# jesselasse/MARL-DMFB

Measured on AMD Instinct MI355X. Metric: env-steps/sec (whole node), 10x10 DMFB 4-droplet fov9, higher is better.
Workload: dtype int8 env state/obs + f64 rewards; fp32 Q-net; 1 GPU; DMFB 10x10, drop_num=4, fov=9, 4096 parallel envs per GPU (BASELINE configs[1]); parallelism=dp1: chips sharded per rank, one flat RCCL all-reduce per learn

## Files before the change

### marl_dmfb_amd/_lib.py

```python
import ctypes as C
import os

_HERE = os.path.dirname(os.path.abspath(__file__))
LIB_DIR = os.path.join(_HERE, 'lib')
_CACHE = {}
_FILE = {'rollout_route': 'rollout_ops'}


class HipLibraryMissing(RuntimeError):
    pass


def load(name):
    if name in _CACHE:
        return _CACHE[name]
    stem = _FILE.get(name, name)
    path = os.path.join(LIB_DIR, 'lib%s%s.so' % (stem, os.environ.get('MARL_DMFB_VARIANT_' + stem.upper(), '')))
    if not os.path.exists(path):
        raise HipLibraryMissing(
            '%s not found: build the HIP extension first (python -c "import __graft_entry__ as g; g.build()" '
            'or make -C marl_dmfb_amd/csrc). There is no CPU fallback.' % path)
    import torch
    lib = C.CDLL(path)
    _CACHE[name] = lib
# ... 169 lines not shown
        'meda_plan_route': [i32, i32, i32, i32, vp, vp, vp, vp, vp, vp, vp, vp, vp, vp],
        'meda_plan_max_dim': ([], i32),
        'meda_plan_lds_bytes': ([i32, i32, i32], i32),
        'meda_plan_last_hip_error': ([], i32),
    },
    'vdn_ops': {
        'vdn_td_forward': [vp, vp, vp, vp, vp, vp, vp, i32, i32, i32, i32, i32, f32, vp, vp, vp, vp],
        'vdn_td_backward': [vp, vp, vp, vp, i32, i32, i32, i32, i32, vp, vp],
        'vdn_td_forward_packed': [vp, vp, vp, i32, vp, vp, vp, vp, vp, i32, i32, f32, vp, vp, vp, vp],
        'vdn_td_backward_packed': [vp, vp, vp, i32, vp, vp, i32, i32, vp, vp],
        'vdn_gather_units': [vp, i32, vp, i32, i32, i32, vp, vp],
        'vdn_clip_adam_step': [i32, C.POINTER(vp), C.POINTER(vp), C.POINTER(vp), C.POINTER(vp), C.POINTER(i64), f32, f64, f64, f64,
                               f64, f64, f64, vp, vp, vp, vp],
        'vdn_last_hip_error': ([], i32),
    },
    'qmix_ops': {
        'qmix_mix_td_forward': [vp, vp, vp, vp, vp, vp, vp, i32, i32, i32, i32, i32, vp, i32, i32, vp, i32, i32, i32, i32,
                                C.POINTER(QmixMixer), C.POINTER(QmixMixer), f32, vp, vp, vp, vp],
        'qmix_mix_td_backward': [vp, vp, vp, vp, i32, i32, i32, i32, i32, vp, i32, i32, i32, i32, C.POINTER(QmixMixer), vp, vp, vp,
                                 vp, vp, vp],
        'qmix_last_hip_error': ([], i32),
    },
}

DMFB_VEC_SYMBOLS = list(SIGNATURES['dmfb_vec'])
MEDA_VEC_SYMBOLS = list(SIGNATURES['meda_vec'])

ENV_ERRORS = {
    'dmfb_vec': {
        -1: (ValueError, 'bad argument'),
# ... 103 lines not shown
    return _library('rollout_route')


def route_plan():
    return _library('route_plan')


def meda_plan():
    return _library('meda_plan')


def vdn_ops():
    return _library('vdn_ops')


def qmix_ops():
    return _library('qmix_ops')
```

### marl_dmfb_amd/csrc/crnn_ops.hip

```cpp
#include <hip/hip_runtime.h>

#include <cstdint>
#include <cstdio>
#include <cstdlib>

#include "../../include/crnn_ops.h"

#define HIP_ABI_TAG "crnn_ops"
#define HIP_ABI_ERR CRNN_ERR_HIP
#include "hip_abi.h"
#include "crnn_mfma.h"
#include "crnn_mfma19.h"
#include "crnn_bwd19.h"

namespace {

constexpr int kBlock = 512;
constexpr int kA1Stride = 52;
constexpr int kDz1Unit = 108;

constexpr int kLdsBudget = 158 * 1024;

template <int OD> struct GeoB {
    static constexpr int DZ2 = 28;
// ... 354 lines not shown
            for (; b + kRedY < n_part; b += 2 * kRedY) { a0 += part[(size_t)b * G::PART + off[k]]; a1 += part[(size_t)(b + kRedY) * G::PART + off[k]]; }
            if (b < n_part) a0 += part[(size_t)b * G::PART + off[k]];
            acc += a0 + a1;
        }
    }
    s_sum[ty][tx] = acc;
    __syncthreads();
    if (ty == 0 && i < n2 + nb + n1 + nb) {
        float t = 0.0f;
#pragma unroll
        for (int k = 0; k < kRedY; ++k) t += s_sum[k][tx];
        grads[i] = t;
    }
}

constexpr int kMlpBlock = 256, kMlpOut = 10, kMlpMaxIn = 18, kMlpMaxParts = 256;
__global__ __launch_bounds__(kMlpBlock) void k_mlp_bwd(const int8_t *__restrict__ obs, long obs_stride, int dir_off,
                                                       const int8_t *__restrict__ onehot, int n_actions, long rows,
                                                       const float *__restrict__ x, long x_stride, const float *__restrict__ g, long g_stride,
                                                       int col0, float *__restrict__ part) {
    __shared__ float s_red[kMlpBlock / 64][kMlpOut * (kMlpMaxIn + 1)];
    float acc[kMlpOut][kMlpMaxIn + 1];
#pragma unroll
    for (int o = 0; o < kMlpOut; ++o)
#pragma unroll
        for (int k = 0; k <= kMlpMaxIn; ++k) acc[o][k] = 0.0f;
    for (long r = (long)blockIdx.x * kMlpBlock + threadIdx.x; r < rows; r += (long)gridDim.x * kMlpBlock) {
        float v[kMlpMaxIn];
        v[0] = (float)obs[r * obs_stride + dir_off];
        v[1] = (float)obs[r * obs_stride + dir_off + 1];
#pragma unroll
        for (int k = 0; k < kMlpMaxIn - 2; ++k) v[2 + k] = k < n_actions ? (float)onehot[r * n_actions + k] : 0.0f;
#pragma unroll
        for (int o = 0; o < kMlpOut; ++o) {
            const float gz = x[r * x_stride + col0 + o] > 0.0f ? g[r * g_stride + col0 + o] : 0.0f;
#pragma unroll
            for (int k = 0; k < kMlpMaxIn; ++k) acc[o][k] = fmaf(gz, v[k], acc[o][k]);
            acc[o][kMlpMaxIn] += gz;
        }
    }
    const int lane = threadIdx.x & 63, wave = threadIdx.x >> 6;
#pragma unroll
    for (int o = 0; o < kMlpOut; ++o)
#pragma unroll
        for (int k = 0; k <= kMlpMaxIn; ++k) {
            float t = acc[o][k];
            for (int d = 32; d > 0; d >>= 1) t += __shfl_xor(t, d);
            if (lane == 0) s_red[wave][o * (kMlpMaxIn + 1) + k] = t;
        }
    __syncthreads();
    for (int i = threadIdx.x; i < kMlpOut * (kMlpMaxIn + 1); i += kMlpBlock) {
        float t = 0.0f;
#pragma unroll
        for (int w = 0; w < kMlpBlock / 64; ++w) t += s_red[w][i];
        part[(size_t)blockIdx.x * kMlpOut * (kMlpMaxIn + 1) + i] = t;
    }
}
__global__ __launch_bounds__(256) void k_mlp_bwd_reduce(const float *__restrict__ part, int n_part, int nin, float *__restrict__ dw, float *__restrict__ db) {
    const int i = threadIdx.x;
    if (i >= kMlpOut * nin + kMlpOut) return;
    const int o = i < kMlpOut * nin ? i / nin : i - kMlpOut * nin, k = i < kMlpOut * nin ? i - o * nin : kMlpMaxIn;
    float t = 0.0f;
    for (int b = 0; b < n_part; ++b) t += part[(size_t)b * kMlpOut * (kMlpMaxIn + 1) + o * (kMlpMaxIn + 1) + k];
    if (i < kMlpOut * nin) dw[i] = t;
    else db[o] = t;
}

struct LiveRows { const int32_t *chips; const int32_t *n; int rows_per_chip; };

template <int OD, int RBV>
int launch_rb(const int8_t *obs, long obs_stride, long rows, const float *w1, const float *b1, const float *w2, const float *b2,
              float *out, long out_stride, int out_cols, const int8_t *onehot, int n_actions, const float *mlp_w, const float *mlp_b, hipStream_t s,
              LiveRows live = LiveRows{nullptr, nullptr, 1}) {
    using GM = crnn_mfma::GeoM<OD, RBV>;
    const size_t lds = GM::LDS_FLOATS * sizeof(float);
    static LdsLimit lds_limit;
    if (const int rc = lds_limit.raise((const void *)crnn_mfma::k_conv9_mfma<OD, RBV>, lds)) return rc;
    const long n_blocks = (rows + GM::RB - 1) / GM::RB;
    const long resident = 256L * (long)((size_t)160 * 1024 / lds);
    const int grid = (int)(n_blocks < resident ? n_blocks : resident);
// ... 128 lines not shown
    if (od == 32) return launch_bwd<32>(d_obs, obs_stride, rows, d_out, out_stride, d_grad_out, grad_stride, d_w2, d_part, n_part, d_grads, d_w1, d_b1, (hipStream_t)stream);
    return CRNN_ERR_UNSUPPORTED;
}

int crnn_mlp_backward_parts(void) { return kMlpMaxParts * kMlpOut * (kMlpMaxIn + 1); }

int crnn_mlp_backward(const int8_t *d_obs, int64_t obs_stride, int dir_offset, const int8_t *d_onehot, int n_actions, int64_t rows,
                      const float *d_out, int64_t out_stride, const float *d_grad_out, int64_t grad_stride, int col0, float *d_part,
                      float *d_grad_w, float *d_grad_b, void *stream) {
    if (!d_obs || !d_onehot || !d_out || !d_grad_out || !d_part || !d_grad_w || !d_grad_b || rows <= 0 || n_actions < 0 ||
        n_actions > kMlpMaxIn - 2 || dir_offset < 0 || obs_stride < dir_offset + 2 || col0 < 0 || out_stride < col0 + kMlpOut ||
        grad_stride < col0 + kMlpOut)
        return CRNN_ERR_BAD_ARG;
    const long want = (rows + kMlpBlock - 1) / kMlpBlock;
    const int grid = (int)(want < kMlpMaxParts ? want : kMlpMaxParts);
    HIP_TRY(launch_status([&] {
        hipLaunchKernelGGL(k_mlp_bwd, dim3(grid), dim3(kMlpBlock), 0, (hipStream_t)stream, d_obs, (long)obs_stride, dir_offset, d_onehot, n_actions,
                           (long)rows, d_out, (long)out_stride, d_grad_out, (long)grad_stride, col0, d_part);
        hipLaunchKernelGGL(k_mlp_bwd_reduce, dim3(1), dim3(256), 0, (hipStream_t)stream, d_part, grid, 2 + n_actions, d_grad_w, d_grad_b);
    }));
    return CRNN_OK;
}

int crnn_conv19_backward_parts(int od) { return od == 24 ? crnn_bwd19::GeoB19<24>::PART : od == 32 ? crnn_bwd19::GeoB19<32>::PART : CRNN_ERR_UNSUPPORTED; }

int crnn_conv19_backward(const int8_t *d_obs, int64_t obs_stride, int64_t rows, const float *d_out, int64_t out_stride,
                         const float *d_grad_out, int64_t grad_stride, const float *d_w1, const float *d_b1, const float *d_w3,
                         const float *d_b3, int od, float *d_part, int n_part, float *d_grads, void *stream) {
    if (!d_obs || !d_out || !d_grad_out || !d_w1 || !d_b1 || !d_w3 || !d_b3 || !d_part || !d_grads || rows <= 0 || n_part < 1 ||
        n_part > 256 || obs_stride < 3 * 19 * 19 || out_stride < od * 25 || grad_stride < od * 25)
        return CRNN_ERR_BAD_ARG;
    if (od == 24) return launch_bwd19<24>(d_obs, obs_stride, rows, d_out, out_stride, d_grad_out, grad_stride, d_w1, d_b1, d_w3, d_b3, d_part, n_part, d_grads, (hipStream_t)stream);
    if (od == 32) return launch_bwd19<32>(d_obs, obs_stride, rows, d_out, out_stride, d_grad_out, grad_stride, d_w1, d_b1, d_w3, d_b3, d_part, n_part, d_grads, (hipStream_t)stream);
    return CRNN_ERR_UNSUPPORTED;
}
// ... 5 lines not shown
```

### marl_dmfb_amd/csrc/hip_abi.h

```cpp
#pragma once

#include <hip/hip_runtime.h>

#include <cstdio>
#include <cstdlib>

#if !defined(HIP_ABI_TAG) || !defined(HIP_ABI_ERR)
#error "define HIP_ABI_TAG and HIP_ABI_ERR before including hip_abi.h"
#endif

namespace {

thread_local int g_last_hip = 0;

inline int hip_fail(hipError_t e, const char *what, int line) {
    g_last_hip = (int)e;
    if (getenv("DMFB_VEC_DEBUG"))
        fprintf(stderr, HIP_ABI_TAG ": %s failed at line %d: %s (%d)\n", what, line, hipGetErrorString(e), (int)e);
    return HIP_ABI_ERR;
}

#define HIP_TRY(expr)                                                 \
    do {                                                              \
        hipError_t _e = (expr);                                       \
// ... 30 lines not shown
};

struct LdsLimit {
    bool done[64] = {};
    int raise(const void *kernel, size_t bytes) {
        int dev = 0;
        (void)hipGetDevice(&dev);
        const bool known = dev >= 0 && dev < 64;
        if (known && done[dev]) return 0;
        HIP_TRY(hipFuncSetAttribute(kernel, hipFuncAttributeMaxDynamicSharedMemorySize, (int)bytes));
        if (known) done[dev] = true;
        return 0;
    }
};

}
```

### marl_dmfb_amd/csrc/vdn_ops.hip

```cpp
#include <hip/hip_runtime.h>

#include <cstdint>

#include "../../include/vdn_ops.h"

#define HIP_ABI_TAG "vdn_ops"
#define HIP_ABI_ERR VDN_ERR_HIP
#include "hip_abi.h"

namespace {

__global__ __launch_bounds__(256) void k_td_forward(const float *__restrict__ qe, const float *__restrict__ qt, const int8_t *__restrict__ u,
                                                    const float *__restrict__ r, const int8_t *__restrict__ avail,
                                                    const uint8_t *__restrict__ term, const uint8_t *__restrict__ padded, int B, int T,
                                                    int Tl, int n, int A, float gamma, float *__restrict__ mtd, float *__restrict__ maskf,
                                                    int32_t *__restrict__ bad) {
    const int idx = blockIdx.x * blockDim.x + threadIdx.x;
    if (idx >= B * T) return;
    const int b = idx / T, t = idx - b * T;
    const size_t ep = (size_t)b * Tl + t;
    const size_t q0 = ((size_t)t * B + b) * n * A;
    float qe_tot = 0.0f, qt_tot = 0.0f;
    bool ok = true;
    for (int i = 0; i < n; ++i) {
        int a_taken = (int)u[ep * n + i];
        if ((unsigned)a_taken >= (unsigned)A) { ok = false; a_taken = 0; }
        qe_tot = qe_tot + qe[q0 + (size_t)i * A + a_taken];
        float m = -3.4e38f;
        for (int a = 0; a < A; ++a) {
            const float v = avail[(ep * n + i) * A + a] == 0 ? -9999999.0f : qt[q0 + (size_t)i * A + a];
            m = v > m ? v : m;
        }
        qt_tot = qt_tot + m;
    }
    const float not_term = 1.0f - (term[ep] ? 1.0f : 0.0f);
    const float target = r[ep] + (gamma * qt_tot) * not_term;
    const float mk = 1.0f - (padded[ep] ? 1.0f : 0.0f);
    mtd[idx] = ok ? mk * (target - qe_tot) : __builtin_nanf("");
    maskf[idx] = mk;
    if (!ok && bad) atomicAdd(bad, 1);
}

__global__ __launch_bounds__(256) void k_td_backward(const float *__restrict__ mtd, const float *__restrict__ maskf, const int8_t *__restrict__ u,
                                                     const float *__restrict__ g, int B, int T, int Tl, int n, int A,
                                                     float *__restrict__ gq) {
    const long row = (long)blockIdx.x * blockDim.x + threadIdx.x;
    if (row >= (long)T * B * n) return;
    const int i = (int)(row % n);
    const long tb = row / n;
    const int b = (int)(tb % B), t = (int)(tb / B);
    const int idx = b * T + t;
    const float d = -((2.0f * mtd[idx]) * maskf[idx]) * g[0];
    const int a_taken = (int)u[((size_t)b * Tl + t) * n + i];
    const bool bad_a = (unsigned)a_taken >= (unsigned)A;
    for (int a = 0; a < A; ++a) gq[row * A + a] = (bad_a || a == a_taken) ? d : 0.0f;
}

__global__ __launch_bounds__(256) void k_td_forward_packed(const float *__restrict__ qe, const float *__restrict__ qt, const int32_t *__restrict__ units,
                                                           int U, const int8_t *__restrict__ u, const float *__restrict__ r,
                                                           const int8_t *__restrict__ avail, const uint8_t *__restrict__ term,
                                                           const uint8_t *__restrict__ padded, int n, int A, float gamma,
                                                           float *__restrict__ mtd, float *__restrict__ maskf, int32_t *__restrict__ bad) {
    const int j = blockIdx.x * blockDim.x + threadIdx.x;
    if (j >= U) return;
    const size_t ep = (size_t)units[j];
    const size_t q0 = (size_t)j * n * A;
    float qe_tot = 0.0f, qt_tot = 0.0f;
    bool ok = true;
    for (int i = 0; i < n; ++i) {
        int a_taken = (int)u[ep * n + i];
        if ((unsigned)a_taken >= (unsigned)A) { ok = false; a_taken = 0; }
        qe_tot = qe_tot + qe[q0 + (size_t)i * A + a_taken];
        float m = -3.4e38f;
        for (int a = 0; a < A; ++a) {
            const float v = avail[(ep * n + i) * A + a] == 0 ? -9999999.0f : qt[q0 + (size_t)i * A + a];
            m = v > m ? v : m;
        }
        qt_tot = qt_tot + m;
    }
    const float not_term = 1.0f - (term[ep] ? 1.0f : 0.0f);
    const float target = r[ep] + (gamma * qt_tot) * not_term;
    const float mk = 1.0f - (padded[ep] ? 1.0f : 0.0f);
    mtd[j] = ok ? mk * (target - qe_tot) : __builtin_nanf("");
    maskf[j] = mk;
    if (!ok && bad) atomicAdd(bad, 1);
}

__global__ __launch_bounds__(256) void k_td_backward_packed(const float *__restrict__ mtd, const float *__restrict__ maskf, const int32_t *__restrict__ units,
                                                            const int8_t *__restrict__ u, const float *__restrict__ g, long rows, int n, int A,
                                                            float *__restrict__ gq) {
    const long row = (long)blockIdx.x * blockDim.x + threadIdx.x;
    if (row >= rows) return;
    const int i = (int)(row % n);
    const long j = row / n;
    const float d = -((2.0f * mtd[j]) * maskf[j]) * g[0];
    const int a_taken = (int)u[(size_t)units[j] * n + i];
    const bool bad_a = (unsigned)a_taken >= (unsigned)A;
    for (int a = 0; a < A; ++a) gq[row * A + a] = (bad_a || a == a_taken) ? d : 0.0f;
}

template <typename V>
__global__ __launch_bounds__(256) void k_gather_units(const V *__restrict__ src, int unit_v, const int32_t *__restrict__ units, int U, int shift,
                                                      int zero_below, V *__restrict__ dst) {
    const long idx = (long)blockIdx.x * blockDim.x + threadIdx.x;
    if (idx >= (long)U * unit_v) return;
    const int j = (int)(idx / unit_v), k = (int)(idx - (long)j * unit_v);
    dst[idx] = j < zero_below ? (V)0 : src[((size_t)units[j] + shift) * unit_v + k];
}

}

namespace {

struct TensorList {
    float *p[VDN_MAX_TENSORS];
    float *g[VDN_MAX_TENSORS];
    float *m[VDN_MAX_TENSORS];
    float *v[VDN_MAX_TENSORS];
    long off[VDN_MAX_TENSORS + 1];
    int n;
};

// ... 80 lines not shown
        tl.v[k] = on ? exp_avg_sq[k] : nullptr;
        tl.off[k + 1] = tl.off[k] + (on ? (long)numel[k] : 0);
    }
    HIP_TRY(launch_status([&] {
        hipLaunchKernelGGL(k_sqnorm_partials, dim3(VDN_NORM_BLOCKS), dim3(256), 0, (hipStream_t)stream, tl, d_partials, d_grad_div);
        const long total = tl.off[n_tensors];
        const int blocks = (int)((total + 1023) / 1024 < 1024 ? (total + 1023) / 1024 : 1024);
        hipLaunchKernelGGL(k_clip_adam, dim3(blocks), dim3(256), 0, (hipStream_t)stream, tl, d_partials, VDN_NORM_BLOCKS, max_norm,
                           (float)((double)lr / bias_correction1), (float)(1.0 - beta1), (float)beta2, (float)(1.0 - beta2), (float)eps,
                           (float)sqrt(bias_correction2), d_total_norm, d_grad_div);
    }));
    return VDN_OK;
}


int vdn_td_forward(const float *d_q_eval, const float *d_q_target, const int8_t *d_u, const float *d_r,
                   const int8_t *d_avail_next, const uint8_t *d_terminated, const uint8_t *d_padded, int32_t B, int32_t T,
                   int32_t t_limit, int32_t n_agents, int32_t n_actions, float gamma, float *d_mtd, float *d_mask, int32_t *d_bad_actions,
                   void *stream) {
    if (!d_q_eval || !d_q_target || !d_u || !d_r || !d_avail_next || !d_terminated || !d_padded || !d_mtd || !d_mask || B < 0 ||
        T < 1 || t_limit < T || n_agents < 1 || n_actions < 1 || n_actions > 127)
        return VDN_ERR_BAD_ARG;
    if (B == 0) return VDN_OK;
    const int total = B * T;
    LAUNCH(k_td_forward, dim3((total + 255) / 256), dim3(256), 0, (hipStream_t)stream, d_q_eval, d_q_target, d_u, d_r,
           d_avail_next, d_terminated, d_padded, B, T, t_limit, n_agents, n_actions, gamma, d_mtd, d_mask, d_bad_actions);
    return VDN_OK;
}

int vdn_td_backward(const float *d_mtd, const float *d_mask, const int8_t *d_u, const float *d_grad_num, int32_t B, int32_t T,
                    int32_t t_limit, int32_t n_agents, int32_t n_actions, float *d_grad_q, void *stream) {
    if (!d_mtd || !d_mask || !d_u || !d_grad_num || !d_grad_q || B < 0 || T < 1 || t_limit < T || n_agents < 1 || n_actions < 1 ||
        n_actions > 127)
        return VDN_ERR_BAD_ARG;
    if (B == 0) return VDN_OK;
    const long rows = (long)T * B * n_agents;
    LAUNCH(k_td_backward, dim3((unsigned)((rows + 255) / 256)), dim3(256), 0, (hipStream_t)stream, d_mtd, d_mask, d_u,
           d_grad_num, B, T, t_limit, n_agents, n_actions, d_grad_q);
    return VDN_OK;
}

int vdn_td_forward_packed(const float *d_q_eval, const float *d_q_target, const int32_t *d_units, int32_t n_units, const int8_t *d_u,
                          const float *d_r, const int8_t *d_avail_next, const uint8_t *d_terminated, const uint8_t *d_padded,
                          int32_t n_agents, int32_t n_actions, float gamma, float *d_mtd, float *d_mask, int32_t *d_bad_actions,
                          void *stream) {
    if (!d_q_eval || !d_q_target || !d_units || !d_u || !d_r || !d_avail_next || !d_terminated || !d_padded || !d_mtd || !d_mask ||
        n_units < 0 || n_agents < 1 || n_actions < 1 || n_actions > 127)
        return VDN_ERR_BAD_ARG;
    if (n_units == 0) return VDN_OK;
    LAUNCH(k_td_forward_packed, dim3((unsigned)((n_units + 255) / 256)), dim3(256), 0, (hipStream_t)stream, d_q_eval, d_q_target,
           d_units, n_units, d_u, d_r, d_avail_next, d_terminated, d_padded, n_agents, n_actions, gamma, d_mtd, d_mask,
           d_bad_actions);
    return VDN_OK;
}

int vdn_td_backward_packed(const float *d_mtd, const float *d_mask, const int32_t *d_units, int32_t n_units, const int8_t *d_u,
                           const float *d_grad_num, int32_t n_agents, int32_t n_actions, float *d_grad_q, void *stream) {
    if (!d_mtd || !d_mask || !d_units || !d_u || !d_grad_num || !d_grad_q || n_units < 0 || n_agents < 1 || n_actions < 1 || n_actions > 127)
        return VDN_ERR_BAD_ARG;
    if (n_units == 0) return VDN_OK;
    const long rows = (long)n_units * n_agents;
    LAUNCH(k_td_backward_packed, dim3((unsigned)((rows + 255) / 256)), dim3(256), 0, (hipStream_t)stream, d_mtd, d_mask, d_units,
           d_u, d_grad_num, rows, n_agents, n_actions, d_grad_q);
    return VDN_OK;
}

int vdn_gather_units(const void *d_src, int32_t unit_bytes, const int32_t *d_units, int32_t n_units, int32_t unit_shift,
                     int32_t zero_below, void *d_dst, void *stream) {
    if (!d_src || !d_units || !d_dst || unit_bytes < 1 || n_units < 0 || zero_below < 0) return VDN_ERR_BAD_ARG;
    if (n_units == 0) return VDN_OK;
    HIP_TRY(launch_status([&] {
        const bool dw = unit_bytes % 4 == 0 && ((size_t)d_src | (size_t)d_dst) % 4 == 0;
        const int uv = dw ? unit_bytes / 4 : unit_bytes;
        const long total = (long)n_units * uv;
        if (dw)
            hipLaunchKernelGGL((k_gather_units<uint32_t>), dim3((unsigned)((total + 255) / 256)), dim3(256), 0, (hipStream_t)stream,
                               (const uint32_t *)d_src, uv, d_units, n_units, unit_shift, zero_below, (uint32_t *)d_dst);
        else
            hipLaunchKernelGGL((k_gather_units<uint8_t>), dim3((unsigned)((total + 255) / 256)), dim3(256), 0, (hipStream_t)stream,
                               (const uint8_t *)d_src, uv, d_units, n_units, unit_shift, zero_below, (uint8_t *)d_dst);
    }));
    return VDN_OK;
}

int vdn_last_hip_error(void) { return g_last_hip; }

}
```

### marl_dmfb_amd/policy/vdn.py

```python
import os

import torch

from ..network.base_net import CRNN, RNN
from ..network.vdn_net import VDNNet


def _t(x, device, dtype):
    if not isinstance(x, torch.Tensor):
        x = torch.as_tensor(x)
    return x.to(device=device, dtype=dtype)


def _episode_slots(t):
    inner = 1
    for k in range(t.dim() - 1, 0, -1):
        if t.stride(k) != inner and t.shape[k] != 1:
            return None
        inner *= t.shape[k]
    per_step = inner // t.shape[1]
    if t.shape[0] == 1:
        return t.shape[1]
    if per_step == 0 or t.stride(0) % per_step or t.stride(0) // per_step < t.shape[1]:
        return None
    return t.stride(0) // per_step


class _TDLoss(torch.autograd.Function):

    @staticmethod
    def forward(ctx, q_eval_tm, q_target_tm, u, r, avail_next, terminated, padded, T, gamma, bad=None):
        from .. import _lib
        lib = _lib.checked('vdn_ops')
        B, n, A = u.shape[0], u.shape[2], avail_next.shape[3]
        t_limit = _episode_slots(u)
        q_eval_tm, q_target_tm = q_eval_tm.contiguous(), q_target_tm.contiguous()
        mtd = torch.empty(B * T, dtype=torch.float32, device=u.device)
        mask = torch.empty(B * T, dtype=torch.float32, device=u.device)
        stream = torch.cuda.current_stream(u.device).cuda_stream
        lib.vdn_td_forward(q_eval_tm.data_ptr(), q_target_tm.data_ptr(), u.data_ptr(), r.data_ptr(),
                           avail_next.data_ptr(), terminated.data_ptr(), padded.data_ptr(), B, T, t_limit, n, A,
                           float(gamma), mtd.data_ptr(), mask.data_ptr(),
                           None if bad is None else bad.data_ptr(), stream)
        ctx.save_for_backward(mtd, mask, u)
        ctx.dims = (B, T, t_limit, n, A)
        num, mask_sum = (mtd * mtd).sum(), mask.sum()
        ctx.mark_non_differentiable(mask_sum)
        return num, mask_sum

    @staticmethod
    def backward(ctx, g_num, _g_mask):
        from .. import _lib
        lib = _lib.checked('vdn_ops')
        mtd, mask, u = ctx.saved_tensors
        B, T, t_limit, n, A = ctx.dims
        gq = torch.empty((T, B * n, A), dtype=torch.float32, device=u.device)
        g = g_num.reshape(1).to(torch.float32).contiguous()
        lib.vdn_td_backward(mtd.data_ptr(), mask.data_ptr(), u.data_ptr(), g.data_ptr(), B, T, t_limit, n, A,
                            gq.data_ptr(), torch.cuda.current_stream(u.device).cuda_stream)
        return gq, None, None, None, None, None, None, None, None, None


class _TDLossPacked(torch.autograd.Function):

    @staticmethod
    def forward(ctx, q_eval, q_target, units, n_units, u, r, avail_next, terminated, padded, n, A, gamma, bad=None):
        from .. import _lib
        lib = _lib.checked('vdn_ops')
        q_eval, q_target = q_eval.contiguous(), q_target.contiguous()
        mtd = torch.empty(n_units, dtype=torch.float32, device=u.device)
        mask = torch.empty(n_units, dtype=torch.float32, device=u.device)
        lib.vdn_td_forward_packed(q_eval.data_ptr(), q_target.data_ptr(), units.data_ptr(), n_units, u.data_ptr(),
                                  r.data_ptr(), avail_next.data_ptr(), terminated.data_ptr(), padded.data_ptr(),
                                  n, A, float(gamma), mtd.data_ptr(), mask.data_ptr(),
                                  None if bad is None else bad.data_ptr(), torch.cuda.current_stream(u.device).cuda_stream)
        ctx.save_for_backward(mtd, mask, units, u)
        ctx.dims = (n_units, n, A, q_eval.shape[0])
        num, mask_sum = (mtd * mtd).sum(), mask.sum()
        ctx.mark_non_differentiable(mask_sum)
        return num, mask_sum

    @staticmethod
    def backward(ctx, g_num, _g_mask):
        from .. import _lib
        lib = _lib.checked('vdn_ops')
        mtd, mask, units, u = ctx.saved_tensors
        n_units, n, A, rows_pad = ctx.dims
        gq = torch.empty((rows_pad, A), dtype=torch.float32, device=u.device)
        gq[n_units * n:].zero_()
        g = g_num.reshape(1).to(torch.float32).contiguous()
        lib.vdn_td_backward_packed(mtd.data_ptr(), mask.data_ptr(), units.data_ptr(), n_units, u.data_ptr(),
                                   g.data_ptr(), n, A, gq.data_ptr(), torch.cuda.current_stream(u.device).cuda_stream)
        return (gq,) + (None,) * 12


PACK_ROWS = 2048


class VDN:
    def __init__(self, args):
        self.args = args
        self.n_actions = args.n_actions
        self.n_agents = args.n_agents
        input_shape = args.obs_shape[-1]
        if args.last_action:
            input_shape += self.n_actions
        if args.reuse_network:
# ... 210 lines not shown

    def learn_packed(self, buffers, idx, lens, train_step, plan=None):
        import numpy as np
        dev, n, A = self.device, self.n_agents, self.n_actions
        B, T_ring, O = len(idx), buffers['o'].shape[1], buffers['o'].shape[-1]
        if plan is None:
            counts, units_np = self.pack_units(idx, lens, T_ring)
            units = torch.from_numpy(units_np).to(dev, non_blocking=True)
        else:
            counts, units = plan
        U = int(units.shape[0])
        V = U * n
        pad = PACK_ROWS if V >= 32768 else 64
        Vp = -(-V // pad) * pad
        from .. import _lib
        lib = _lib.checked('vdn_ops')
        stream = torch.cuda.current_stream(dev).cuda_stream

        def packed(src, shift=0, zero_below=0):
            row = src.shape[-1]
            out = torch.empty((Vp, row), dtype=src.dtype, device=dev)
            out[V:].zero_()
            lib.vdn_gather_units(src.data_ptr(), n * row * src.element_size(), units.data_ptr(), U, shift,
                                 zero_below, out.data_ptr(), stream)
            return out
        obs_e, obs_t, oh_t = packed(buffers['o']), packed(buffers['o_next']), packed(buffers['u_onehot'])
        oh_e = packed(buffers['u_onehot'], shift=-1, zero_below=B)
        x_e = self._features(self.eval_rnn, obs_e, oh_e)
        with torch.no_grad():
            x_t = self._features(self.target_rnn, obs_t, oh_t)
        step_rows = [int(c) * n for c in counts]
        if os.environ.get('MARL_DMFB_GRU_PAIR', '1') != '0' and hasattr(self.eval_rnn, 'recurrent_seq_packed_pair'):
            q_e, q_t = self.eval_rnn.recurrent_seq_packed_pair(self.eval_rnn, x_e, self.target_rnn, x_t, step_rows, B * n)
        else:
            q_e = self.eval_rnn.recurrent_seq_packed(x_e, step_rows, B * n)
            with torch.no_grad():
                q_t = self.target_rnn.recurrent_seq_packed(x_t, step_rows, B * n)
        if self._td_bad is None:
            self._td_bad = torch.zeros(1, dtype=torch.int32, device=dev)
        num, mask_sum = _TDLossPacked.apply(q_e, q_t, units, U, buffers['u'], buffers['r'], buffers['avail_u_next'],
                                            buffers['terminated'], buffers['padded'], n, A, self.args.gamma, self._td_bad)
        return self._backward_and_step(num, mask_sum, train_step)
# ... 149 lines not shown
```

Measured before the change: 7.362 million env-steps/s.

## Fuse VDN learn tail reductions, pad zeroing, and unit gathers into fewer kernels

New measurement: 7.498 million env-steps/s (median of 6 runs). Within noise of the previous version (+1.8%).

```diff
diff --git a/include/vdn_tail.h b/include/vdn_tail.h
--- /dev/null
+++ b/include/vdn_tail.h
@@ -0,0 +1,32 @@
+#ifndef VDN_TAIL_H
+#define VDN_TAIL_H
+
+#include <stdint.h>
+
+#ifdef __cplusplus
+extern "C" {
+#endif
+
+int vdn_td_sum_parts(int64_t n_slots);
+int vdn_td_forward_sums(const float *d_q_eval, const float *d_q_target, const int8_t *d_u, const float *d_r,
+                        const int8_t *d_avail_next, const uint8_t *d_terminated, const uint8_t *d_padded, int32_t B, int32_t T,
+                        int32_t t_limit, int32_t n_agents, int32_t n_actions, float gamma, float *d_mtd, float *d_mask,
+                        int32_t *d_bad_actions, float *d_part, float *d_sums, void *stream);
+int vdn_td_forward_packed_sums(const float *d_q_eval, const float *d_q_target, const int32_t *d_units, int32_t n_units,
+                               const int8_t *d_u, const float *d_r, const int8_t *d_avail_next, const uint8_t *d_terminated,
+                               const uint8_t *d_padded, int32_t n_agents, int32_t n_actions, float gamma, float *d_mtd, float *d_mask,
+                               int32_t *d_bad_actions, float *d_part, float *d_sums, void *stream);
+
+int vdn_td_backward_packed_pad(const float *d_mtd, const float *d_mask, const int32_t *d_units, int32_t n_units, const int8_t *d_u,
+                               const float *d_grad_num, int32_t n_agents, int32_t n_actions, int64_t rows_pad, float *d_grad_q,
+                               void *stream);
+
+#define VDN_GATHER_MAX 4
+int vdn_gather_units_batch(int32_t n_gathers, const void *const *d_src, const int32_t *unit_bytes, const int32_t *unit_shift,
+                           const int32_t *zero_below, void *const *d_dst, const int64_t *dst_bytes, const int32_t *d_units,
+                           int32_t n_units, void *stream);
+
+#ifdef __cplusplus
+}
+#endif
+#endif
diff --git a/marl_dmfb_amd/_lib.py b/marl_dmfb_amd/_lib.py
--- a/marl_dmfb_amd/_lib.py
+++ b/marl_dmfb_amd/_lib.py
@@ -4,7 +4,7 @@
 _HERE = os.path.dirname(os.path.abspath(__file__))
 LIB_DIR = os.path.join(_HERE, 'lib')
 _CACHE = {}
-_FILE = {'rollout_route': 'rollout_ops'}
+_FILE = {'rollout_route': 'rollout_ops', 'vdn_tail': 'vdn_ops'}
 
 
 class HipLibraryMissing(RuntimeError):
@@ -207,6 +207,14 @@
                                f64, f64, f64, vp, vp, vp, vp],
         'vdn_last_hip_error': ([], i32),
     },
+    'vdn_tail': {
+        'vdn_td_sum_parts': ([i64], i32),
+        'vdn_td_forward_sums': [vp, vp, vp, vp, vp, vp, vp, i32, i32, i32, i32, i32, f32, vp, vp, vp, vp, vp, vp],
+        'vdn_td_forward_packed_sums': [vp, vp, vp, i32, vp, vp, vp, vp, vp, i32, i32, f32, vp, vp, vp, vp, vp, vp],
+        'vdn_td_backward_packed_pad': [vp, vp, vp, i32, vp, vp, i32, i32, i64, vp, vp],
+        'vdn_gather_units_batch': [i32, C.POINTER(vp), C.POINTER(i32), C.POINTER(i32), C.POINTER(i32), C.POINTER(vp), C.POINTER(i64), vp,
+                                   i32, vp],
+    },
     'qmix_ops': {
         'qmix_mix_td_forward': [vp, vp, vp, vp, vp, vp, vp, i32, i32, i32, i32, i32, vp, i32, i32, vp, i32, i32, i32, i32,
                                 C.POINTER(QmixMixer), C.POINTER(QmixMixer), f32, vp, vp, vp, vp],
@@ -340,5 +348,9 @@
     return _library('vdn_ops')
 
 
+def vdn_tail():
+    return _library('vdn_tail')
+
+
 def qmix_ops():
     return _library('qmix_ops')
diff --git a/marl_dmfb_amd/csrc/crnn_ops.hip b/marl_dmfb_amd/csrc/crnn_ops.hip
--- a/marl_dmfb_amd/csrc/crnn_ops.hip
+++ b/marl_dmfb_amd/csrc/crnn_ops.hip
@@ -392,12 +392,15 @@
     }
 }
 
-constexpr int kMlpBlock = 256, kMlpOut = 10, kMlpMaxIn = 18, kMlpMaxParts = 256;
+constexpr int kMlpBlock = 256, kMlpOut = 10, kMlpMaxIn = 18, kMlpMaxParts = 256, kMlpTailLoads = 64;
+__device__ unsigned g_mlp_ticket = 0;
 __global__ __launch_bounds__(kMlpBlock) void k_mlp_bwd(const int8_t *__restrict__ obs, long obs_stride, int dir_off,
                                                        const int8_t *__restrict__ onehot, int n_actions, long rows,
                                                        const float *__restrict__ x, long x_stride, const float *__restrict__ g, long g_stride,
-                                                       int col0, float *__restrict__ part) {
+                                                       int col0, float *part, float *__restrict__ dw, float *__restrict__ db) {
     __shared__ float s_red[kMlpBlock / 64][kMlpOut * (kMlpMaxIn + 1)];
+    __shared__ int s_last;
+    const int nin = 2 + n_actions, n_part = (int)gridDim.x;
     float acc[kMlpOut][kMlpMaxIn + 1];
 #pragma unroll
     for (int o = 0; o < kMlpOut; ++o)
@@ -413,7 +416,8 @@
         for (int o = 0; o < kMlpOut; ++o) {
             const float gz = x[r * x_stride + col0 + o] > 0.0f ? g[r * g_stride + col0 + o] : 0.0f;
 #pragma unroll
-            for (int k = 0; k < kMlpMaxIn; ++k) acc[o][k] = fmaf(gz, v[k], acc[o][k]);
+            for (int k = 0; k < kMlpMaxIn; ++k)
+                if (k < nin) acc[o][k] = fmaf(gz, v[k], acc[o][k]);
             acc[o][kMlpMaxIn] += gz;
         }
     }
@@ -421,27 +425,36 @@
 #pragma unroll
     for (int o = 0; o < kMlpOut; ++o)
 #pragma unroll
-        for (int k = 0; k <= kMlpMaxIn; ++k) {
-            float t = acc[o][k];
-            for (int d = 32; d > 0; d >>= 1) t += __shfl_xor(t, d);
-            if (lane == 0) s_red[wave][o * (kMlpMaxIn + 1) + k] = t;
-        }
+        for (int k = 0; k <= kMlpMaxIn; ++k)
+            if (k < nin || k == kMlpMaxIn) {
+                float t = acc[o][k];
+                for (int d = 32; d > 0; d >>= 1) t += __shfl_xor(t, d);
+                if (lane == 0) s_red[wave][o * (kMlpMaxIn + 1) + k] = t;
+            }
     __syncthreads();
-    for (int i = threadIdx.x; i < kMlpOut * (kMlpMaxIn + 1); i += kMlpBlock) {
+    const int n_out = kMlpOut * (nin + 1);
+    for (int i = threadIdx.x; i < n_out; i += kMlpBlock) {
+        const int o = i < kMlpOut * nin ? i / nin : i - kMlpOut * nin, k = i < kMlpOut * nin ? i - o * nin : kMlpMaxIn;
         float t = 0.0f;
 #pragma unroll
-        for (int w = 0; w < kMlpBlock / 64; ++w) t += s_red[w][i];
-        part[(size_t)blockIdx.x * kMlpOut * (kMlpMaxIn + 1) + i] = t;
-    }
-}
-__global__ __launch_bounds__(256) void k_mlp_bwd_reduce(const float *__restrict__ part, int n_part, int nin, float *__restrict__ dw, float *__restrict__ db) {
-    const int i = threadIdx.x;
-    if (i >= kMlpOut * nin + kMlpOut) return;
-    const int o = i < kMlpOut * nin ? i / nin : i - kMlpOut * nin, k = i < kMlpOut * nin ? i - o * nin : kMlpMaxIn;
-    float t = 0.0f;
-    for (int b = 0; b < n_part; ++b) t += part[(size_t)b * kMlpOut * (kMlpMaxIn + 1) + o * (kMlpMaxIn + 1) + k];
-    if (i < kMlpOut * nin) dw[i] = t;
-    else db[o] = t;
+        for (int w = 0; w < kMlpBlock / 64; ++w) t += s_red[w][o * (kMlpMaxIn + 1) + k];
+        part[(size_t)i * n_part + blockIdx.x] = t;
+    }
+    if (!last_workgroup_arrives(&g_mlp_ticket, gridDim.x, &s_last)) return;
+    for (int i = threadIdx.x; i < n_out; i += kMlpBlock) {
+        const float *p = part + (size_t)i * n_part;
+        float t = 0.0f;
+        for (int b0 = 0; b0 < n_part; b0 += kMlpTailLoads) {
+            float v[kMlpTailLoads];
+#pragma unroll
+            for (int u = 0; u < kMlpTailLoads; ++u) v[u] = b0 + u < n_part ? partial_load(p + b0 + u) : 0.0f;
+#pragma unroll
+            for (int u = 0; u < kMlpTailLoads; ++u)
+                if (b0 + u < n_part) t += v[u];
+        }
+        if (i < kMlpOut * nin) dw[i] = t;
+        else db[i - kMlpOut * nin] = t;
+    }
 }
 
 struct LiveRows { const int32_t *chips; const int32_t *n; int rows_per_chip; };
@@ -600,11 +613,8 @@
         return CRNN_ERR_BAD_ARG;
     const long want = (rows + kMlpBlock - 1) / kMlpBlock;
     const int grid = (int)(want < kMlpMaxParts ? want : kMlpMaxParts);
-    HIP_TRY(launch_status([&] {
-        hipLaunchKernelGGL(k_mlp_bwd, dim3(grid), dim3(kMlpBlock), 0, (hipStream_t)stream, d_obs, (long)obs_stride, dir_offset, d_onehot, n_actions,
-                           (long)rows, d_out, (long)out_stride, d_grad_out, (long)grad_stride, col0, d_part);
-        hipLaunchKernelGGL(k_mlp_bwd_reduce, dim3(1), dim3(256), 0, (hipStream_t)stream, d_part, grid, 2 + n_actions, d_grad_w, d_grad_b);
-    }));
+    LAUNCH(k_mlp_bwd, dim3(grid), dim3(kMlpBlock), 0, (hipStream_t)stream, d_obs, (long)obs_stride, dir_offset, d_onehot, n_actions,
+           (long)rows, d_out, (long)out_stride, d_grad_out, (long)grad_stride, col0, d_part, d_grad_w, d_grad_b);
     return CRNN_OK;
 }
 
diff --git a/marl_dmfb_amd/csrc/hip_abi.h b/marl_dmfb_amd/csrc/hip_abi.h
--- a/marl_dmfb_amd/csrc/hip_abi.h
+++ b/marl_dmfb_amd/csrc/hip_abi.h
@@ -68,4 +68,25 @@
     }
 };
 
+__device__ __forceinline__ bool last_workgroup_arrives(unsigned *ticket, unsigned n_groups, int *s_last) {
+    asm volatile("s_waitcnt vmcnt(0)" ::: "memory");
+    __syncthreads();
+    if (threadIdx.x == 0) {
+        __builtin_amdgcn_fence(__ATOMIC_RELEASE, "agent");
+        asm volatile("s_waitcnt vmcnt(0)" ::: "memory");
+        const bool last = atomicInc(ticket, n_groups - 1) == n_groups - 1;
+        if (last) {
+            __builtin_amdgcn_fence(__ATOMIC_ACQUIRE, "agent");
+            asm volatile("s_waitcnt vmcnt(0)" ::: "memory");
+        }
+        *s_last = last ? 1 : 0;
+    }
+    __syncthreads();
+    return *s_last != 0;
 }
+
+__device__ __forceinline__ float partial_load(const float *p) {
+    return __hip_atomic_load(p, __ATOMIC_RELAXED, __HIP_MEMORY_SCOPE_AGENT);
+}
+
+}
diff --git a/marl_dmfb_amd/csrc/vdn_ops.hip b/marl_dmfb_amd/csrc/vdn_ops.hip
--- a/marl_dmfb_amd/csrc/vdn_ops.hip
+++ b/marl_dmfb_amd/csrc/vdn_ops.hip
@@ -3,20 +3,40 @@
 #include <cstdint>
 
 #include "../../include/vdn_ops.h"
+#include "../../include/vdn_tail.h"
 
 #define HIP_ABI_TAG "vdn_ops"
 #define HIP_ABI_ERR VDN_ERR_HIP
 #include "hip_abi.h"
 
 namespace {
+
+__device__ unsigned g_td_ticket = 0;
+__device__ __forceinline__ void td_block_sums(float sq, float mk, float *part, float *__restrict__ sums) {
+    __shared__ float s_w[2][4];
+    __shared__ int s_last;
+    for (int o = 32; o > 0; o >>= 1) { sq += __shfl_xor(sq, o); mk += __shfl_xor(mk, o); }
+    if ((threadIdx.x & 63) == 0) { s_w[0][threadIdx.x >> 6] = sq; s_w[1][threadIdx.x >> 6] = mk; }
+    __syncthreads();
+    if (threadIdx.x < 2) part[2 * blockIdx.x + threadIdx.x] = (s_w[threadIdx.x][0] + s_w[threadIdx.x][1]) + (s_w[threadIdx.x][2] + s_w[threadIdx.x][3]);
+    if (!last_workgroup_arrives(&g_td_ticket, gridDim.x, &s_last)) return;
+    if (threadIdx.x < 128) {
+        const int which = threadIdx.x >> 6;
+        float t = 0.0f;
+        for (unsigned b = threadIdx.x & 63; b < gridDim.x; b += 64) t += partial_load(part + 2 * b + which);
+        for (int o = 32; o > 0; o >>= 1) t += __shfl_xor(t, o);
+        if ((threadIdx.x & 63) == 0) sums[which] = t;
+    }
+}
 
 __global__ __launch_bounds__(256) void k_td_forward(const float *__restrict__ qe, const float *__restrict__ qt, const int8_t *__restrict__ u,
                                                     const float *__restrict__ r, const int8_t *__restrict__ avail,
                                                     const uint8_t *__restrict__ term, const uint8_t *__restrict__ padded, int B, int T,
                                                     int Tl, int n, int A, float gamma, float *__restrict__ mtd, float *__restrict__ maskf,
-                                                    int32_t *__restrict__ bad) {
+                                                    int32_t *__restrict__ bad, float *part, float *__restrict__ sums) {
     const int idx = blockIdx.x * blockDim.x + threadIdx.x;
-    if (idx >= B * T) return;
+    float sq = 0.0f, mks = 0.0f;
+    if (idx < B * T) {
     const int b = idx / T, t = idx - b * T;
     const size_t ep = (size_t)b * Tl + t;
     const size_t q0 = ((size_t)t * B + b) * n * A;
@@ -36,9 +56,14 @@
     const float not_term = 1.0f - (term[ep] ? 1.0f : 0.0f);
     const float target = r[ep] + (gamma * qt_tot) * not_term;
     const float mk = 1.0f - (padded[ep] ? 1.0f : 0.0f);
-    mtd[idx] = ok ? mk * (target - qe_tot) : __builtin_nanf("");
+    const float m = ok ? mk * (target - qe_tot) : __builtin_nanf("");
+    mtd[idx] = m;
     maskf[idx] = mk;
     if (!ok && bad) atomicAdd(bad, 1);
+    sq = m * m;
+    mks = mk;
+    }
+    if (sums) td_block_sums(sq, mks, part, sums);
 }
 
 __global__ __launch_bounds__(256) void k_td_backward(const float *__restrict__ mtd, const float *__restrict__ maskf, const int8_t *__restrict__ u,
@@ -60,9 +85,11 @@
                                                            int U, const int8_t *__restrict__ u, const float *__restrict__ r,
                                                            const int8_t *__restrict__ avail, const uint8_t *__restrict__ term,
                                                            const uint8_t *__restrict__ padded, int n, int A, float gamma,
-                                                           float *__restrict__ mtd, float *__restrict__ maskf, int32_t *__restrict__ bad) {
+                                                           float *__restrict__ mtd, float *__restrict__ maskf, int32_t *__restrict__ bad,
+                                                           float *part, float *__restrict__ sums) {
     const int j = blockIdx.x * blockDim.x + threadIdx.x;
-    if (j >= U) return;
+    float sq = 0.0f, mks = 0.0f;
+    if (j < U) {
     const size_t ep = (size_t)units[j];
     const size_t q0 = (size_t)j * n * A;
     float qe_tot = 0.0f, qt_tot = 0.0f;
@@ -81,16 +108,25 @@
     const float not_term = 1.0f - (term[ep] ? 1.0f : 0.0f);
     const float target = r[ep] + (gamma * qt_tot) * not_term;
     const float mk = 1.0f - (padded[ep] ? 1.0f : 0.0f);
-    mtd[j] = ok ? mk * (target - qe_tot) : __builtin_nanf("");
+    const float m = ok ? mk * (target - qe_tot) : __builtin_nanf("");
+    mtd[j] = m;
     maskf[j] = mk;
     if (!ok && bad) atomicAdd(bad, 1);
+    sq = m * m;
+    mks = mk;
+    }
+    if (sums) td_block_sums(sq, mks, part, sums);
 }
 
 __global__ __launch_bounds__(256) void k_td_backward_packed(const float *__restrict__ mtd, const float *__restrict__ maskf, const int32_t *__restrict__ units,
-                                                            const int8_t *__restrict__ u, const float *__restrict__ g, long rows, int n, int A,
-                                                            float *__restrict__ gq) {
+                                                            const int8_t *__restrict__ u, const float *__restrict__ g, long rows, long rows_pad,
+                                                            int n, int A, float *__restrict__ gq) {
     const long row = (long)blockIdx.x * blockDim.x + threadIdx.x;
-    if (row >= rows) return;
+    if (row >= rows_pad) return;
+    if (row >= rows) {
+        for (int a = 0; a < A; ++a) gq[row * A + a] = 0.0f;
+        return;
+    }
     const int i = (int)(row % n);
     const long j = row / n;
     const float d = -((2.0f * mtd[j]) * maskf[j]) * g[0];
@@ -106,6 +142,30 @@
     if (idx >= (long)U * unit_v) return;
     const int j = (int)(idx / unit_v), k = (int)(idx - (long)j * unit_v);
     dst[idx] = j < zero_below ? (V)0 : src[((size_t)units[j] + shift) * unit_v + k];
+}
+
+struct GatherBatch {
+    const void *src[VDN_GATHER_MAX];
+    void *dst[VDN_GATHER_MAX];
+    long total[VDN_GATHER_MAX], total_pad[VDN_GATHER_MAX];
+    int unit_v[VDN_GATHER_MAX], shift[VDN_GATHER_MAX], zero_below[VDN_GATHER_MAX], dw[VDN_GATHER_MAX];
+};
+template <typename V>
+__device__ __forceinline__ void gather_word(const void *src, int unit_v, const int32_t *__restrict__ units, int shift, int zero_below,
+                                            void *dst, long total, long idx) {
+    V v = (V)0;
+    if (idx < total) {
+        const int j = (int)(idx / unit_v), k = (int)(idx - (long)j * unit_v);
+        if (j >= zero_below) v = ((const V *)src)[((size_t)units[j] + shift) * unit_v + k];
+    }
+    ((V *)dst)[idx] = v;
+}
+__global__ __launch_bounds__(256) void k_gather_units_batch(GatherBatch gb, const int32_t *__restrict__ units) {
+    const int d = blockIdx.y;
+    const long idx = (long)blockIdx.x * blockDim.x + threadIdx.x;
+    if (idx >= gb.total_pad[d]) return;
+    if (gb.dw[d]) gather_word<uint32_t>(gb.src[d], gb.unit_v[d], units, gb.shift[d], gb.zero_below[d], gb.dst[d], gb.total[d], idx);
+    else gather_word<uint8_t>(gb.src[d], gb.unit_v[d], units, gb.shift[d], gb.zero_below[d], gb.dst[d], gb.total[d], idx);
 }
 
 }
@@ -216,18 +276,31 @@
 }
 
 
+int vdn_td_sum_parts(int64_t n_slots) { return n_slots < 1 ? 2 : (int)(2 * ((n_slots + 255) / 256)); }
+
+int vdn_td_forward_sums(const float *d_q_eval, const float *d_q_target, const int8_t *d_u, const float *d_r,
+                        const int8_t *d_avail_next, const uint8_t *d_terminated, const uint8_t *d_padded, int32_t B, int32_t T,
+                        int32_t t_limit, int32_t n_agents, int32_t n_actions, float gamma, float *d_mtd, float *d_mask,
+                        int32_t *d_bad_actions, float *d_part, float *d_sums, void *stream) {
+    if ((d_sums && !d_part) || !d_q_eval || !d_q_target || !d_u || !d_r || !d_avail_next || !d_terminated || !d_padded || !d_mtd || !d_mask || B < 0 ||
+        T < 1 || t_limit < T || n_agents < 1 || n_actions < 1 || n_actions > 127)
+        return VDN_ERR_BAD_ARG;
+    if (B == 0) {
+        if (d_sums) HIP_TRY(hipMemsetAsync(d_sums, 0, 2 * sizeof(float), (hipStream_t)stream));
+        return VDN_OK;
+    }
+    const int total = B * T;
+    LAUNCH(k_td_forward, dim3((total + 255) / 256), dim3(256), 0, (hipStream_t)stream, d_q_eval, d_q_target, d_u, d_r,
+           d_avail_next, d_terminated, d_padded, B, T, t_limit, n_agents, n_actions, gamma, d_mtd, d_mask, d_bad_actions, d_part, d_sums);
+    return VDN_OK;
+}
+
 int vdn_td_forward(const float *d_q_eval, const float *d_q_target, const int8_t *d_u, const float *d_r,
                    const int8_t *d_avail_next, const uint8_t *d_terminated, const uint8_t *d_padded, int32_t B, int32_t T,
                    int32_t t_limit, int32_t n_agents, int32_t n_actions, float gamma, float *d_mtd, float *d_mask, int32_t *d_bad_actions,
                    void *stream) {
-    if (!d_q_eval || !d_q_target || !d_u || !d_r || !d_avail_next || !d_terminated || !d_padded || !d_mtd || !d_mask || B < 0 ||
-        T < 1 || t_limit < T || n_agents < 1 || n_actions < 1 || n_actions > 127)
-        return VDN_ERR_BAD_ARG;
-    if (B == 0) return VDN_OK;
-    const int total = B * T;
-    LAUNCH(k_td_forward, dim3((total + 255) / 256), dim3(256), 0, (hipStream_t)stream, d_q_eval, d_q_target, d_u, d_r,
-           d_avail_next, d_terminated, d_padded, B, T, t_limit, n_agents, n_actions, gamma, d_mtd, d_mask, d_bad_actions);
-    return VDN_OK;
+    return vdn_td_forward_sums(d_q_eval, d_q_target, d_u, d_r, d_avail_next, d_terminated, d_padded, B, T, t_limit, n_agents, n_actions,
+                               gamma, d_mtd, d_mask, d_bad_actions, nullptr, nullptr, stream);
 }
 
 int vdn_td_backward(const float *d_mtd, const float *d_mask, const int8_t *d_u, const float *d_grad_num, int32_t B, int32_t T,
@@ -242,29 +315,48 @@
     return VDN_OK;
 }
 
+int vdn_td_forward_packed_sums(const float *d_q_eval, const float *d_q_target, const int32_t *d_units, int32_t n_units,
+                               const int8_t *d_u, const float *d_r, const int8_t *d_avail_next, const uint8_t *d_terminated,
+                               const uint8_t *d_padded, int32_t n_agents, int32_t n_actions, float gamma, float *d_mtd, float *d_mask,
+                               int32_t *d_bad_actions, float *d_part, float *d_sums, void *stream) {
+    if ((d_sums && !d_part) || !d_q_eval || !d_q_target || !d_units || !d_u || !d_r || !d_avail_next || !d_terminated || !d_padded || !d_mtd || !d_mask ||
+        n_units < 0 || n_agents < 1 || n_actions < 1 || n_actions > 127)
+        return VDN_ERR_BAD_ARG;
+    if (n_units == 0) {
+        if (d_sums) HIP_TRY(hipMemsetAsync(d_sums, 0, 2 * sizeof(float), (hipStream_t)stream));
+        return VDN_OK;
+    }
+    LAUNCH(k_td_forward_packed, dim3((unsigned)((n_units + 255) / 256)), dim3(256), 0, (hipStream_t)stream, d_q_eval, d_q_target,
+           d_units, n_units, d_u, d_r, d_avail_next, d_terminated, d_padded, n_agents, n_actions, gamma, d_mtd, d_mask,
+           d_bad_actions, d_part, d_sums);
+    return VDN_OK;
+}
+
 int vdn_td_forward_packed(const float *d_q_eval, const float *d_q_target, const int32_t *d_units, int32_t n_units, const int8_t *d_u,
                           const float *d_r, const int8_t *d_avail_next, const uint8_t *d_terminated, const uint8_t *d_padded,
                           int32_t n_agents, int32_t n_actions, float gamma, float *d_mtd, float *d_mask, int32_t *d_bad_actions,
                           void *stream) {
-    if (!d_q_eval || !d_q_target || !d_units || !d_u || !d_r || !d_avail_next || !d_terminated || !d_padded || !d_mtd || !d_mask ||
-        n_units < 0 || n_agents < 1 || n_actions < 1 || n_actions > 127)
-        return VDN_ERR_BAD_ARG;
-    if (n_units == 0) return VDN_OK;
-    LAUNCH(k_td_forward_packed, dim3((unsigned)((n_units + 255) / 256)), dim3(256), 0, (hipStream_t)stream, d_q_eval, d_q_target,
-           d_units, n_units, d_u, d_r, d_avail_next, d_terminated, d_padded, n_agents, n_actions, gamma, d_mtd, d_mask,
-           d_bad_actions);
+    return vdn_td_forward_packed_sums(d_q_eval, d_q_target, d_units, n_units, d_u, d_r, d_avail_next, d_terminated, d_padded, n_agents,
+                                      n_actions, gamma, d_mtd, d_mask, d_bad_actions, nullptr, nullptr, stream);
+}
+
+int vdn_td_backward_packed_pad(const float *d_mtd, const float *d_mask, const int32_t *d_units, int32_t n_units, const int8_t *d_u,
+                               const float *d_grad_num, int32_t n_agents, int32_t n_actions, int64_t rows_pad, float *d_grad_q,
+                               void *stream) {
+    if (!d_mtd || !d_mask || !d_units || !d_u || !d_grad_num || !d_grad_q || n_units < 0 || n_agents < 1 || n_actions < 1 ||
+        n_actions > 127 || rows_pad < (int64_t)n_units * n_agents)
+        return VDN_ERR_BAD_ARG;
+    if (rows_pad == 0) return VDN_OK;
+    const long rows = (long)n_units * n_agents;
+    LAUNCH(k_td_backward_packed, dim3((unsigned)((rows_pad + 255) / 256)), dim3(256), 0, (hipStream_t)stream, d_mtd, d_mask, d_units,
+           d_u, d_grad_num, rows, (long)rows_pad, n_agents, n_actions, d_grad_q);
     return VDN_OK;
 }
 
 int vdn_td_backward_packed(const float *d_mtd, const float *d_mask, const int32_t *d_units, int32_t n_units, const int8_t *d_u,
                            const float *d_grad_num, int32_t n_agents, int32_t n_actions, float *d_grad_q, void *stream) {
-    if (!d_mtd || !d_mask || !d_units || !d_u || !d_grad_num || !d_grad_q || n_units < 0 || n_agents < 1 || n_actions < 1 || n_actions > 127)
-        return VDN_ERR_BAD_ARG;
-    if (n_units == 0) return VDN_OK;
-    const long rows = (long)n_units * n_agents;
-    LAUNCH(k_td_backward_packed, dim3((unsigned)((rows + 255) / 256)), dim3(256), 0, (hipStream_t)stream, d_mtd, d_mask, d_units,
-           d_u, d_grad_num, rows, n_agents, n_actions, d_grad_q);
-    return VDN_OK;
+    return vdn_td_backward_packed_pad(d_mtd, d_mask, d_units, n_units, d_u, d_grad_num, n_agents, n_actions, (int64_t)n_units * n_agents,
+                                      d_grad_q, stream);
 }
 
 int vdn_gather_units(const void *d_src, int32_t unit_bytes, const int32_t *d_units, int32_t n_units, int32_t unit_shift,
@@ -285,6 +377,34 @@
     return VDN_OK;
 }
 
+int vdn_gather_units_batch(int32_t n_gathers, const void *const *d_src, const int32_t *unit_bytes, const int32_t *unit_shift,
+                           const int32_t *zero_below, void *const *d_dst, const int64_t *dst_bytes, const int32_t *d_units,
+                           int32_t n_units, void *stream) {
+    if (n_gathers < 1 || n_gathers > VDN_GATHER_MAX || !d_src || !unit_bytes || !unit_shift || !zero_below || !d_dst || !dst_bytes ||
+        !d_units || n_units < 0)
+        return VDN_ERR_BAD_ARG;
+    GatherBatch gb{};
+    long most = 0;
+    for (int i = 0; i < n_gathers; ++i) {
+        if (!d_src[i] || !d_dst[i] || unit_bytes[i] < 1 || zero_below[i] < 0 || dst_bytes[i] < (int64_t)n_units * unit_bytes[i])
+            return VDN_ERR_BAD_ARG;
+        const bool dw = unit_bytes[i] % 4 == 0 && dst_bytes[i] % 4 == 0 && ((size_t)d_src[i] | (size_t)d_dst[i]) % 4 == 0;
+        gb.src[i] = d_src[i];
+        gb.dst[i] = d_dst[i];
+        gb.dw[i] = dw ? 1 : 0;
+        gb.unit_v[i] = dw ? unit_bytes[i] / 4 : unit_bytes[i];
+        gb.total[i] = (long)n_units * gb.unit_v[i];
+        gb.total_pad[i] = (long)(dw ? dst_bytes[i] / 4 : dst_bytes[i]);
+        gb.shift[i] = unit_shift[i];
+        gb.zero_below[i] = zero_below[i];
+        most = gb.total_pad[i] > most ? gb.total_pad[i] : most;
+    }
+    if (most == 0) return VDN_OK;
+    if ((most + 255) / 256 > 0x7fffffffL) return VDN_ERR_BAD_ARG;
+    LAUNCH(k_gather_units_batch, dim3((unsigned)((most + 255) / 256), (unsigned)n_gathers), dim3(256), 0, (hipStream_t)stream, gb, d_units);
+    return VDN_OK;
+}
+
 int vdn_last_hip_error(void) { return g_last_hip; }
 
 }
diff --git a/marl_dmfb_amd/policy/vdn.py b/marl_dmfb_amd/policy/vdn.py
--- a/marl_dmfb_amd/policy/vdn.py
+++ b/marl_dmfb_amd/policy/vdn.py
@@ -31,20 +31,22 @@
     @staticmethod
     def forward(ctx, q_eval_tm, q_target_tm, u, r, avail_next, terminated, padded, T, gamma, bad=None):
         from .. import _lib
-        lib = _lib.checked('vdn_ops')
+        lib = _lib.checked('vdn_tail')
         B, n, A = u.shape[0], u.shape[2], avail_next.shape[3]
         t_limit = _episode_slots(u)
         q_eval_tm, q_target_tm = q_eval_tm.contiguous(), q_target_tm.contiguous()
         mtd = torch.empty(B * T, dtype=torch.float32, device=u.device)
         mask = torch.empty(B * T, dtype=torch.float32, device=u.device)
+        part = torch.empty(lib.vdn_td_sum_parts(B * T), dtype=torch.float32, device=u.device)
+        sums = torch.empty(2, dtype=torch.float32, device=u.device)
         stream = torch.cuda.current_stream(u.device).cuda_stream
-        lib.vdn_td_forward(q_eval_tm.data_ptr(), q_target_tm.data_ptr(), u.data_ptr(), r.data_ptr(),
-                           avail_next.data_ptr(), terminated.data_ptr(), padded.data_ptr(), B, T, t_limit, n, A,
-                           float(gamma), mtd.data_ptr(), mask.data_ptr(),
-                           None if bad is None else bad.data_ptr(), stream)
+        lib.vdn_td_forward_sums(q_eval_tm.data_ptr(), q_target_tm.data_ptr(), u.data_ptr(), r.data_ptr(),
+                                avail_next.data_ptr(), terminated.data_ptr(), padded.data_ptr(), B, T, t_limit, n, A,
+                                float(gamma), mtd.data_ptr(), mask.data_ptr(),
+                                None if bad is None else bad.data_ptr(), part.data_ptr(), sums.data_ptr(), stream)
         ctx.save_for_backward(mtd, mask, u)
         ctx.dims = (B, T, t_limit, n, A)
-        num, mask_sum = (mtd * mtd).sum(), mask.sum()
+        num, mask_sum = sums[0], sums[1]
         ctx.mark_non_differentiable(mask_sum)
         return num, mask_sum
 
@@ -66,31 +68,33 @@
     @staticmethod
     def forward(ctx, q_eval, q_target, units, n_units, u, r, avail_next, terminated, padded, n, A, gamma, bad=None):
         from .. import _lib
-        lib = _lib.checked('vdn_ops')
+        lib = _lib.checked('vdn_tail')
         q_eval, q_target = q_eval.contiguous(), q_target.contiguous()
         mtd = torch.empty(n_units, dtype=torch.float32, device=u.device)
         mask = torch.empty(n_units, dtype=torch.float32, device=u.device)
-        lib.vdn_td_forward_packed(q_eval.data_ptr(), q_target.data_ptr(), units.data_ptr(), n_units, u.data_ptr(),
-                                  r.data_ptr(), avail_next.data_ptr(), terminated.data_ptr(), padded.data_ptr(),
-                                  n, A, float(gamma), mtd.data_ptr(), mask.data_ptr(),
-                                  None if bad is None else bad.data_ptr(), torch.cuda.current_stream(u.device).cuda_stream)
+        part = torch.empty(lib.vdn_td_sum_parts(n_units), dtype=torch.float32, device=u.device)
+        sums = torch.empty(2, dtype=torch.float32, device=u.device)
+        lib.vdn_td_forward_packed_sums(q_eval.data_ptr(), q_target.data_ptr(), units.data_ptr(), n_units, u.data_ptr(),
+                                       r.data_ptr(), avail_next.data_ptr(), terminated.data_ptr(), padded.data_ptr(),
+                                       n, A, float(gamma), mtd.data_ptr(), mask.data_ptr(),
+                                       None if bad is None else bad.data_ptr(), part.data_ptr(), sums.data_ptr(),
+                                       torch.cuda.current_stream(u.device).cuda_stream)
         ctx.save_for_backward(mtd, mask, units, u)
         ctx.dims = (n_units, n, A, q_eval.shape[0])
-        num, mask_sum = (mtd * mtd).sum(), mask.sum()
+        num, mask_sum = sums[0], sums[1]
         ctx.mark_non_differentiable(mask_sum)
         return num, mask_sum
 
     @staticmethod
     def backward(ctx, g_num, _g_mask):
         from .. import _lib
-        lib = _lib.checked('vdn_ops')
+        lib = _lib.checked('vdn_tail')
         mtd, mask, units, u = ctx.saved_tensors
         n_units, n, A, rows_pad = ctx.dims
         gq = torch.empty((rows_pad, A), dtype=torch.float32, device=u.device)
-        gq[n_units * n:].zero_()
         g = g_num.reshape(1).to(torch.float32).contiguous()
-        lib.vdn_td_backward_packed(mtd.data_ptr(), mask.data_ptr(), units.data_ptr(), n_units, u.data_ptr(),
-                                   g.data_ptr(), n, A, gq.data_ptr(), torch.cuda.current_stream(u.device).cuda_stream)
+        lib.vdn_td_backward_packed_pad(mtd.data_ptr(), mask.data_ptr(), units.data_ptr(), n_units, u.data_ptr(),
+                                       g.data_ptr(), n, A, rows_pad, gq.data_ptr(), torch.cuda.current_stream(u.device).cuda_stream)
         return (gq,) + (None,) * 12
 
 
@@ -331,18 +335,18 @@
         pad = PACK_ROWS if V >= 32768 else 64
         Vp = -(-V // pad) * pad
         from .. import _lib
-        lib = _lib.checked('vdn_ops')
+        import ctypes as C
+        lib = _lib.checked('vdn_tail')
         stream = torch.cuda.current_stream(dev).cuda_stream
-
-        def packed(src, shift=0, zero_below=0):
-            row = src.shape[-1]
-            out = torch.empty((Vp, row), dtype=src.dtype, device=dev)
-            out[V:].zero_()
-            lib.vdn_gather_units(src.data_ptr(), n * row * src.element_size(), units.data_ptr(), U, shift,
-                                 zero_below, out.data_ptr(), stream)
-            return out
-        obs_e, obs_t, oh_t = packed(buffers['o']), packed(buffers['o_next']), packed(buffers['u_onehot'])
-        oh_e = packed(buffers['u_onehot'], shift=-1, zero_below=B)
+        jobs = [(buffers['o'], 0, 0), (buffers['o_next'], 0, 0), (buffers['u_onehot'], 0, 0), (buffers['u_onehot'], -1, B)]
+        outs = [torch.empty((Vp, src.shape[-1]), dtype=src.dtype, device=dev) for src, _, _ in jobs]
+        k = len(jobs)
+        lib.vdn_gather_units_batch(k, (C.c_void_p * k)(*[src.data_ptr() for src, _, _ in jobs]),
+                                   (C.c_int32 * k)(*[n * src.shape[-1] * src.element_size() for src, _, _ in jobs]),
+                                   (C.c_int32 * k)(*[shift for _, shift, _ in jobs]), (C.c_int32 * k)(*[zb for _, _, zb in jobs]),
+                                   (C.c_void_p * k)(*[out.data_ptr() for out in outs]),
+                                   (C.c_int64 * k)(*[out.numel() * out.element_size() for out in outs]), units.data_ptr(), U, stream)
+        obs_e, obs_t, oh_t, oh_e = outs
         x_e = self._features(self.eval_rnn, obs_e, oh_e)
         with torch.no_grad():
             x_t = self._features(self.target_rnn, obs_t, oh_t)
```
